# nihui/rife-ncnn-vulkan

Measured on AMD Instinct MI355X. Metric: interpolated frames/sec (rife-v4.6, 3840x2160), higher is better.
Workload: dtype f16x2-split MFMA + f32 accumulate (fp32-equivalent; activations stored f32 or as {hi, lo} f16 pairs); 1 GPU; rife-v4.6 3840x2160 frame pairs resident in HBM, timestep sweep [0.5, 0.125, 0.25, 0.7, 0.9], synthetic seeded weights; pairs_in_flight_per_gpu=4, cu_partition=every stream owns 1 / 2 of the compute units (rife_hip_stream_create), frames=F1: images/0.png, 1.png of the reference tiled 6 x 6, parallelism=frame pairs sharded over ranks, no data-path collective

## Files before the change

### rife-ncnn-vulkan_amd/csrc/conv_rs.h

```cpp
#pragma once
#include <type_traits>
#include "conv_t64.h"
#include "conv_row.h"

namespace rife {

constexpr int RS_NR = 12;
constexpr int RS_SEG = 34 * 32;
constexpr int RS_ROWB = 8 * RS_SEG;
constexpr int RS_STG_ROW = 8 * 1024;
constexpr int RS_LDS_RING = 0;
constexpr int RS_LDS_STG = RS_NR * RS_ROWB;
constexpr int RS_NSTG = 3;
constexpr int RS_LDS_BS = RS_LDS_STG + RS_NSTG * 2 * RS_STG_ROW;
constexpr int RS_LDS = RS_LDS_BS + 512;
constexpr int RS_AHEAD = 3;
constexpr int RS_MIN_PAIRS = 4;
constexpr int RS_NTHR = 512;

struct RsArgs {
    const unsigned char* in;
    unsigned char* out;
    const unsigned char* img;
    int H, W;
    int pitch;
    unsigned plane;
    int npairs;
    int nunits;
    int descend;
    long long* stamps = nullptr;
};
enum { RS_NOSTORE = 0x100, RS_NODMA = 0x200, RS_NOMATH = 0x400, RS_CLK = 0x40000, RS_PRIO = 0x2000, RS_NTLOAD = 0x4000, RS_NTSTORE = 0x8000 };

struct RsCursor {
    int strip, p;
    __device__ __forceinline__ void init(int u, int npairs) { strip = u / npairs; p = u - strip * npairs; }
    __device__ __forceinline__ bool advance(int npairs, int descend) {
        if (descend) { if (--p < 0) { p = npairs - 1; --strip; return true; } }
        else if (++p >= npairs) { p = 0; ++strip; return true; }
        return false;
    }
};

template <int TAG>
__device__ __forceinline__ void rs_dma16(const unsigned char* base, unsigned voff, unsigned dst) {
    unsigned keep;
    if RIFE_ABL(TAG & RS_NTLOAD)
        asm volatile("s_mov_b32 %0, m0\n\ts_mov_b32 m0, %2\n\ts_nop 0\n\tglobal_load_lds_dwordx4 %1, %3 nt\n\ts_mov_b32 m0, %0"
                     : "=&s"(keep) : "v"(voff), "s"(dst), "s"(base) : "memory");
    else
        asm volatile("s_mov_b32 %0, m0\n\ts_mov_b32 m0, %2\n\ts_nop 0\n\tglobal_load_lds_dwordx4 %1, %3\n\ts_mov_b32 m0, %0"
                     : "=&s"(keep) : "v"(voff), "s"(dst), "s"(base) : "memory");
}

#define RS_SYNC_LGKM() asm volatile("s_waitcnt lgkmcnt(0)\n\ts_barrier" ::: "memory")
#define RS_SYNC_VM(N) asm volatile("s_waitcnt vmcnt(" #N ")\n\ts_barrier" ::: "memory")
#define RS_SYNC_BARE() asm volatile("s_barrier" ::: "memory")

struct RsPairDesc { int c, t; bool idn; };
__host__ __device__ constexpr RsPairDesc rs_pair(int N, int m) {
    for (int c = 0; c < 4; c++) {
        const int cnt = 9 + ((c >> 1) == N ? 1 : 0);
        if (m < cnt) return m < 9 ? RsPairDesc{c, m, false} : RsPairDesc{c, 4, true};
        m -= cnt;
    }
    return RsPairDesc{0, 0, false};
}
constexpr int RS_NPAIR = 38, RS_PF = 3;

template <int N, int TAG>
__device__ __forceinline__ void rs_consumer(const RsArgs& a, unsigned char* const ldsb, const int ro, const int lane, const int S, const int ufirst) {
    const int h = lane >> 5, li = lane & 31;
    constexpr bool FAST = (TAG & S16_FAST) != 0;
    f16x8 W[4][9];
    {
        const unsigned char* wsrc = a.img + h * 1024 + (N * 32 + li) * 16;
#pragma unroll
        for (int c = 0; c < 4; c++)
#pragma unroll
            for (int t = 0; t < 9; t++) W[c][t] = *reinterpret_cast<const f16x8*>(wsrc + c * t64_wch(2) + t * 2048);
    }
    f16x8 idf[2];
    {
        const int ch = s16_row_channel(li);
#pragma unroll
        for (int hc = 0; hc < 2; hc++)
#pragma unroll
            for (int e = 0; e < 8; e++) idf[hc][e] = ch == 16 * hc + 8 * h + e ? (_Float16)1.f : (_Float16)0.f;
    }
    unsigned colo[3];
#pragma unroll
    for (int dx = 0; dx < 3; dx++) { const int px = li + dx; colo[dx] = (unsigned)(px * 32 + ((h ^ ((px >> 3) & 1)) << 4)); }
    unsigned char* const stg = ldsb + RS_LDS_STG + ro * RS_STG_ROW + ((2 * N + h) * 32 + li) * 64;
    const int qs = (li >> 1) & 3;

    RsCursor cur; cur.init(ufirst, a.npairs);
    int sq = 0;
    unsigned ad[9];
    auto step_addresses = [&](const bool fresh) {
        sq += fresh ? 4 : 2; if (sq >= RS_NR) sq -= RS_NR;
#pragma unroll
        for (int dy = 0; dy < 3; dy++) {
            const int j = ro + dy;
            int sl = a.descend ? sq + RS_NR - 1 - j : sq + RS_NR - 4 + j;
            if (sl >= RS_NR) sl -= RS_NR;
            const unsigned rb = (unsigned)(RS_LDS_RING + sl * RS_ROWB);
#pragma unroll
            for (int dx = 0; dx < 3; dx++) ad[dy * 3 + dx] = rb + colo[dx];
        }
    };
    constexpr int NF = RS_PF + 1;
    static_assert(NF == 4 && RS_NPAIR % NF == 2, "fragment set rotation across steps");
    f16x8 fh[NF], fl[NF];
    int it = 0;
    auto step = [&](auto par_c) {
        constexpr int PAR = decltype(par_c)::value;
        auto frag_read = [&](auto mc) {
            constexpr int m = decltype(mc)::value;
            constexpr RsPairDesc d = rs_pair(N, m % RS_NPAIR);
            constexpr int st = (m + 2 * PAR) % NF;
            fh[st] = *reinterpret_cast<const f16x8*>(ldsb + ad[d.t] + d.c * (2 * RS_SEG));
            if constexpr (!FAST || d.idn) fl[st] = *reinterpret_cast<const f16x8*>(ldsb + ad[d.t] + d.c * (2 * RS_SEG) + RS_SEG);
        };
        f32x16 accH, accL;
        if (!RIFE_ABL(TAG & RS_NOMATH)) {
            for_each_slot<0, RS_NPAIR>([&](auto mc) {
                constexpr int m = decltype(mc)::value;
                constexpr RsPairDesc d = rs_pair(N, m);
                constexpr int st = (m + 2 * PAR) % NF;
                if constexpr (m == RS_NPAIR - RS_PF) step_addresses(cur.advance(a.npairs, a.descend));
                frag_read(std::integral_constant<int, m + RS_PF>{});
                const f16x8 A = d.idn ? idf[d.c & 1] : W[d.c][d.t];
                if constexpr (FAST) {
                    if constexpr (m == 0) {
                        f32x16 z;
#pragma unroll
                        for (int q = 0; q < 16; q++) z[q] = 0.f;
                        accH = __builtin_amdgcn_mfma_f32_32x32x16_f16(A, fh[st], z, 0, 0, 0);
                    } else accH = __builtin_amdgcn_mfma_f32_32x32x16_f16(A, fh[st], accH, 0, 0, 0);
                    if constexpr (d.idn && (d.c & 1) == 0) {
                        f32x16 z;
#pragma unroll
                        for (int q = 0; q < 16; q++) z[q] = 0.f;
                        accL = __builtin_amdgcn_mfma_f32_32x32x16_f16(A, fl[st], z, 0, 0, 0);
                    } else if constexpr (d.idn) accL = __builtin_amdgcn_mfma_f32_32x32x16_f16(A, fl[st], accL, 0, 0, 0);
                } else
                if constexpr (m == 0) {
                    f32x16 z;
#pragma unroll
                    for (int q = 0; q < 16; q++) z[q] = 0.f;
                    accH = __builtin_amdgcn_mfma_f32_32x32x16_f16(A, fh[st], z, 0, 0, 0);
                    accL = __builtin_amdgcn_mfma_f32_32x32x16_f16(A, fl[st], z, 0, 0, 0);
                } else {
                    accH = __builtin_amdgcn_mfma_f32_32x32x16_f16(A, fh[st], accH, 0, 0, 0);
                    accL = __builtin_amdgcn_mfma_f32_32x32x16_f16(A, fl[st], accL, 0, 0, 0);
                }
                __builtin_amdgcn_sched_barrier(0);
            });
        } else {
#pragma unroll
            for (int q = 0; q < 16; q++) { accH[q] = (float)lane; accL[q] = 0.f; }
        }
        int sb = it % RS_NSTG;
        f32x4* const d4 = reinterpret_cast<f32x4*>(stg + sb * (2 * RS_STG_ROW));
#pragma unroll
        for (int q = 0; q < 4; q++) {
            f32x4 v;
#pragma unroll
            for (int k = 0; k < 4; k++) v[k] = accH[4 * q + k] + accL[4 * q + k];
            d4[q ^ qs] = v;
        }
        RS_SYNC_BARE();
        it++;
    };
    RS_SYNC_LGKM();
    step_addresses(true);
    if (!RIFE_ABL(TAG & RS_NOMATH)) for_each_slot<0, RS_PF>([&](auto mc) {
        constexpr int m = decltype(mc)::value;
        constexpr RsPairDesc d = rs_pair(N, m);
        fh[m % NF] = *reinterpret_cast<const f16x8*>(ldsb + ad[d.t] + d.c * (2 * RS_SEG));
        if constexpr (!FAST || d.idn) fl[m % NF] = *reinterpret_cast<const f16x8*>(ldsb + ad[d.t] + d.c * (2 * RS_SEG) + RS_SEG);
    });
    while (it + 1 < S) { step(std::integral_constant<int, 0>{}); step(std::integral_constant<int, 1>{}); }
    if (it < S) step(std::integral_constant<int, 0>{});
    RS_SYNC_LGKM();
}

template <int TAG, int SPLIT = 0>
__global__ __launch_bounds__(RS_NTHR) __attribute__((amdgpu_waves_per_eu(2, 2))) void conv_rs_kernel(RsArgs a) {
    extern __shared__ __attribute__((aligned(16))) unsigned char ldsb[];
    const int tid = threadIdx.x, lane = tid & 63;
    const int wv = __builtin_amdgcn_readfirstlane(tid >> 6);
    long long clk0 = 0, rt0 = 0;
    if RIFE_ABL(TAG & RS_CLK) { clk0 = (long long)__builtin_readcyclecounter(); rt0 = (long long)__builtin_amdgcn_s_memrealtime(); }

    const int nwg = gridDim.x, b = blockIdx.x;
    const int u0 = (int)((long long)a.nunits * b / nwg), u1 = (int)((long long)a.nunits * (b + 1) / nwg);
    const int S = u1 - u0;
    if (S <= 0) return;
    const int ufirst = a.descend ? u1 - 1 : u0;

    auto epilogue = [&](const int j, const int sb, const int cstrip, const int cp, const int cc0, const int cc1, const float slope) {
        const int px = lane >> 1, jh = lane & 1, qs = (px >> 1) & 3;
        const int y = 2 * cp + j, x0 = 32 * cstrip;
        if (!(y < a.H) || RIFE_ABL(TAG & RS_NOSTORE)) return;
        const unsigned okmask = x0 + px < a.W ? 0xffffffffu : 0u;
        const unsigned char* src = ldsb + RS_LDS_STG + sb * (2 * RS_STG_ROW) + j * RS_STG_ROW + px * 64;
        unsigned char* dst = a.out + ((unsigned)((y + 1) * a.pitch + x0 + 1) * 32u + (unsigned)(lane * 16));
        for (int cc = cc0; cc < cc1; cc++) {
            const f32x4 r0 = *reinterpret_cast<const f32x4*>(src + cc * 2048 + (((2 * jh) ^ qs) << 4));
            const f32x4 r1 = *reinterpret_cast<const f32x4*>(src + cc * 2048 + (((2 * jh + 1) ^ qs) << 4));
            const f32x4 b0 = *reinterpret_cast<const f32x4*>(ldsb + RS_LDS_BS + (16 * cc + 8 * jh) * 4);
            const f32x4 b1 = *reinterpret_cast<const f32x4*>(ldsb + RS_LDS_BS + (16 * cc + 8 * jh + 4) * 4);
            f16x8 hv, lv;
#pragma unroll
            for (int e = 0; e < 8; e++) {
                const float yv = (e < 4 ? r0[e & 3] : r1[e & 3]) + (e < 4 ? b0[e & 3] : b1[e & 3]);
                float v = yv < 0.f ? yv * slope : yv;
                v = __uint_as_float(__float_as_uint(v) & okmask);
                const _Float16 hh = (_Float16)v;
                hv[e] = hh;
                lv[e] = (_Float16)(v - (float)hh);
            }
            *reinterpret_cast<f16x8*>(dst + (size_t)(2 * cc) * a.plane) = hv;
            *reinterpret_cast<f16x8*>(dst + (size_t)(2 * cc + 1) * a.plane) = lv;
        }
    };
    if (wv < 4) {
        if RIFE_ABL(TAG & RS_PRIO) __builtin_amdgcn_s_setprio(2);
        if (wv == 0 && lane < 32) reinterpret_cast<f32x4*>(ldsb + RS_LDS_BS)[lane] = reinterpret_cast<const f32x4*>(a.img + 4 * t64_wch(2))[lane];
        if (wv & 1) rs_consumer<1, TAG>(a, ldsb, wv >> 1, lane, S, ufirst);
        else rs_consumer<0, TAG>(a, ldsb, wv >> 1, lane, S, ufirst);
    } else if (wv < 6) {
        const int j = wv - 4;
        unsigned soff[9];
#pragma unroll
        for (int i = 0; i < 9; i++) {
            const int u = min(i * 64 + lane, 543);
            const int seg = u / 68, within = u - seg * 68;
            const int px = within >> 1, pos = within & 1;
            const int kh = pos ^ ((px >> 3) & 1);
            soff[i] = (unsigned)seg * a.plane + (unsigned)(px * 32 + kh * 16);
        }
        RsCursor cur; cur.init(ufirst, a.npairs);
        int sq = 0;
        auto load_step = [&](bool fresh) -> int {
            const int nnew = fresh ? 4 : 2;
            const int y = 2 * cur.p, x0 = 32 * cur.strip;
            int mine = 0;
            for (int i = j; i < nnew; i += 2) {
                const int prow = a.descend ? y + nnew - 1 - i : y + 4 - nnew + i;
                int sl = sq + i; if (sl >= RS_NR) sl -= RS_NR;
                if (!RIFE_ABL(TAG & RS_NODMA)) {
                    const unsigned rowoff = (unsigned)(prow * a.pitch + x0) * 32u;
                    const unsigned dst = (unsigned)(RS_LDS_RING + sl * RS_ROWB);
#pragma unroll
                    for (int k = 0; k < 8; k++) rs_dma16<TAG>(a.in, rowoff + soff[k], dst + k * 1024);
                    if (lane < 32) rs_dma16<TAG>(a.in, rowoff + soff[8], dst + 8 * 1024);
                }
                mine += 9;
            }
            sq += nnew; if (sq >= RS_NR) sq -= RS_NR;
            return mine;
        };
        if RIFE_ABL(TAG & RS_NODMA) { for (int i = lane + 64 * j; i < RS_LDS_STG / 16; i += 128) reinterpret_cast<f32x4*>(ldsb)[i] = f32x4{0.f, 0.f, 0.f, 0.f}; }
        load_step(true);
        int ahead = 0;
        int loaded = 1;
        for (; loaded < RS_AHEAD && loaded < S; loaded++) { const bool f = cur.advance(a.npairs, a.descend); ahead = load_step(f); }
        if (loaded < RS_AHEAD) ahead = 0;
#define RS_WAIT_AHEAD()                                                                                      \
        if RIFE_ABL(TAG & RS_NODMA) RS_SYNC_LGKM();                                                                  \
        else if (ahead == 0) RS_SYNC_VM(0);                                                                  \
        else if (ahead == 9) RS_SYNC_VM(9);                                                                  \
        else RS_SYNC_VM(18);
        RS_WAIT_AHEAD()
        if (SPLIT) {
            const float slope = reinterpret_cast<const float*>(a.img + 4 * t64_wch(2))[64];
            RsCursor ecur; ecur.init(ufirst, a.npairs);
            for (int it = 0; it <= S + 1; it++) {
                if (it >= 2) { epilogue(j, (it - 2) % RS_NSTG, ecur.strip, ecur.p, 0, 2, slope); ecur.advance(a.npairs, a.descend); }
                if (it < S) {
                    if (it + RS_AHEAD < S) { const bool f = cur.advance(a.npairs, a.descend); ahead = load_step(f); }
                    else ahead = 0;
                    asm volatile("s_waitcnt lgkmcnt(0)" ::: "memory");
                    RS_WAIT_AHEAD()
                } else if (it == S) RS_SYNC_LGKM();
            }
        } else {
        for (int it = 0; it < S; it++) {
            if (it + RS_AHEAD < S) { const bool f = cur.advance(a.npairs, a.descend); ahead = load_step(f); }
            else ahead = 0;
            RS_WAIT_AHEAD()
        }
        RS_SYNC_BARE();
        }
#undef RS_WAIT_AHEAD
    } else {
        const int j = wv - 6;
        const int px = lane >> 1, jh = lane & 1, qs = (px >> 1) & 3;
        const float slope = reinterpret_cast<const float*>(a.img + 4 * t64_wch(2))[64];
        RsCursor cur; cur.init(ufirst, a.npairs);
        RS_SYNC_LGKM();
        for (int it = 0; it <= S + 1; it++) {
            if (it >= 2) {
                const int y = 2 * cur.p + j, x0 = 32 * cur.strip;
                if (SPLIT) epilogue(j, (it - 2) % RS_NSTG, cur.strip, cur.p, 2, 4, slope);
                else if (y < a.H && !RIFE_ABL(TAG & RS_NOSTORE)) {
                    const unsigned okmask = x0 + px < a.W ? 0xffffffffu : 0u;
                    const unsigned char* src = ldsb + RS_LDS_STG + ((it - 2) % RS_NSTG) * (2 * RS_STG_ROW) + j * RS_STG_ROW + px * 64;
                    unsigned char* dst = a.out + ((unsigned)((y + 1) * a.pitch + x0 + 1) * 32u + (unsigned)(lane * 16));
#pragma unroll
                    for (int cc = 0; cc < 4; cc++) {
                        const f32x4 r0 = *reinterpret_cast<const f32x4*>(src + cc * 2048 + (((2 * jh) ^ qs) << 4));
                        const f32x4 r1 = *reinterpret_cast<const f32x4*>(src + cc * 2048 + (((2 * jh + 1) ^ qs) << 4));
                        const f32x4 b0 = *reinterpret_cast<const f32x4*>(ldsb + RS_LDS_BS + (16 * cc + 8 * jh) * 4);
                        const f32x4 b1 = *reinterpret_cast<const f32x4*>(ldsb + RS_LDS_BS + (16 * cc + 8 * jh + 4) * 4);
                        f16x8 hv, lv;
#pragma unroll
                        for (int e = 0; e < 8; e++) {
                            const float yv = (e < 4 ? r0[e & 3] : r1[e & 3]) + (e < 4 ? b0[e & 3] : b1[e & 3]);
                            float v = yv < 0.f ? yv * slope : yv;
                            v = __uint_as_float(__float_as_uint(v) & okmask);
                            const _Float16 hh = (_Float16)v;
                            hv[e] = hh;
                            lv[e] = (_Float16)(v - (float)hh);
                        }
                        if RIFE_ABL(TAG & RS_NTSTORE) {
                            __builtin_nontemporal_store(hv, reinterpret_cast<f16x8*>(dst + (size_t)(2 * cc) * a.plane));
                            __builtin_nontemporal_store(lv, reinterpret_cast<f16x8*>(dst + (size_t)(2 * cc + 1) * a.plane));
                        } else {
                            *reinterpret_cast<f16x8*>(dst + (size_t)(2 * cc) * a.plane) = hv;
                            *reinterpret_cast<f16x8*>(dst + (size_t)(2 * cc + 1) * a.plane) = lv;
                        }
                    }
                }
                cur.advance(a.npairs, a.descend);
            }
            if (it < S) RS_SYNC_LGKM();
            else if (it == S) RS_SYNC_LGKM();
        }
    }
    if (RIFE_ABL(TAG & RS_CLK) && tid == 0) {
        a.stamps[4 * blockIdx.x] = (long long)__builtin_readcyclecounter() - clk0;
        a.stamps[4 * blockIdx.x + 1] = rt0;
        a.stamps[4 * blockIdx.x + 2] = (long long)__builtin_amdgcn_s_memrealtime();
    }
}

}
```

### rife-ncnn-vulkan_amd/csrc/conv_rs2.h

```cpp
#pragma once
#include "conv_rs.h"

namespace rife {

constexpr int RS2_SW = 30;
constexpr int RS2_NRA = 8;
constexpr int RS2_NRB = 5;
constexpr int RS2_AH = 3;
constexpr int RS2_NSTG = 3;
constexpr int RS2_LDS_RA = 0;
constexpr int RS2_LDS_RB = RS2_LDS_RA + RS2_NRA * RS_ROWB;
constexpr int RS2_LDS_SA = RS2_LDS_RB + RS2_NRB * RS_ROWB;
constexpr int RS2_LDS_SB = RS2_LDS_SA + RS2_NSTG * RS_STG_ROW;
constexpr int RS2_LDS_BS = RS2_LDS_SB + RS2_NSTG * RS_STG_ROW;
constexpr int RS2_LDS = RS2_LDS_BS + 1024;
static_assert(RS2_LDS <= 160 * 1024, "LDS budget of one CU");
static_assert(RS2_NRA == 4 + RS2_AH + 1, "the row issued in iteration it (sequence it + 4 + AH) takes the slot of row it - 1");
constexpr int RS2_NTHR = 512;
constexpr int RS2_MIN_ROWS = 8;

struct Rs2Args {
    const unsigned char* in;
    unsigned char* out;
    const unsigned char* imgA;
    const unsigned char* imgB;
    int H, W;
    int pitch;
    unsigned plane;
    int rowmax;
    int kparts;
    int nseg;
    int descend;
    int limit;
    long long* stamps = nullptr;
    int stamp_wg = 0;
};

struct Rs2Seg { int x0, ystart, dir, R; };
__device__ __forceinline__ Rs2Seg rs2_segment(const Rs2Args& a, const int seg) {
    const int strip = seg / a.kparts, part = seg - strip * a.kparts;
    const int r0 = (int)((long long)a.H * part / a.kparts), r1 = (int)((long long)a.H * (part + 1) / a.kparts);
    Rs2Seg s;
    s.x0 = RS2_SW * strip; s.R = r1 - r0; s.dir = a.descend ? -1 : 1; s.ystart = a.descend ? r1 - 1 : r0;
    return s;
}

#define RS2_NEXT(V, MOD) { V = V + 1 == (MOD) ? 0 : V + 1; }
enum { RS2_STAMPS = 0x1000, RS2_NOFRAG = 0x10, RS2_NOLO = 0x20 };
constexpr int RS2_NSTAMP = 128;
#define RS2_BAR(KIND)                                                                                                  \
    {                                                                                                                  \
        if (RIFE_ABL(TAG & RS2_STAMPS) && (int)blockIdx.x == a.stamp_wg && bar < RS2_NSTAMP && (threadIdx.x & 63) == 0)         \
            a.stamps[((threadIdx.x >> 6) * RS2_NSTAMP + bar) * 2] = (long long)__builtin_readcyclecounter();           \
        RS_SYNC_##KIND;                                                                                                \
        if (RIFE_ABL(TAG & RS2_STAMPS) && (int)blockIdx.x == a.stamp_wg && bar < RS2_NSTAMP && (threadIdx.x & 63) == 0)         \
            a.stamps[((threadIdx.x >> 6) * RS2_NSTAMP + bar) * 2 + 1] = (long long)__builtin_readcyclecounter();       \
        bar++;                                                                                                         \
    }

template <int N, int NR, int TAG>
__device__ __forceinline__ void rs2_consumer(const Rs2Args& a, const unsigned char* const img, unsigned char* const ldsb, const unsigned ring, const unsigned stgbase,
                                             const int lead, const int extra, const int lag, const int lane) {
    const int h = lane >> 5, li = lane & 31;
    constexpr bool FAST = (TAG & S16_FAST) != 0;
    f16x8 W[4][9];
    {
        const unsigned char* wsrc = img + h * 1024 + (N * 32 + li) * 16;
#pragma unroll
        for (int c = 0; c < 4; c++)
#pragma unroll
            for (int t = 0; t < 9; t++) W[c][t] = *reinterpret_cast<const f16x8*>(wsrc + c * t64_wch(2) + t * 2048);
    }
    f16x8 idf[2];
    {
        const int ch = s16_row_channel(li);
#pragma unroll
        for (int hc = 0; hc < 2; hc++)
#pragma unroll
            for (int e = 0; e < 8; e++) idf[hc][e] = ch == 16 * hc + 8 * h + e ? (_Float16)1.f : (_Float16)0.f;
    }
    unsigned colo[3];
#pragma unroll
    for (int dx = 0; dx < 3; dx++) { const int px = li + dx; colo[dx] = (unsigned)(px * 32 + ((h ^ ((px >> 3) & 1)) << 4)); }
    unsigned char* const stg = ldsb + stgbase + ((2 * N + h) * 32 + li) * 64;
    const int qs = (li >> 1) & 3;

    int bar = 0;
    int sq = 0;
    int sbuf = 0;
    unsigned ad[9];
    auto step_addresses = [&]() {
#pragma unroll
        for (int dy = 0; dy < 3; dy++) {
            int sl = sq + (a.descend ? 2 - dy : dy);
            if (sl >= NR) sl -= NR;
            const unsigned rb = ring + (unsigned)(sl * RS_ROWB);
#pragma unroll
            for (int dx = 0; dx < 3; dx++) ad[dy * 3 + dx] = rb + colo[dx];
        }
    };
    constexpr int NF = RS_PF + 1;
    static_assert(NF == 4 && RS_NPAIR % NF == 2, "fragment set rotation across steps");
    f16x8 fh[NF], fl[NF];
    auto step = [&](auto par_c) {
        constexpr int PAR = decltype(par_c)::value;
        auto frag_read = [&](auto mc) {
            constexpr int m = decltype(mc)::value;
            constexpr RsPairDesc d = rs_pair(N, m % RS_NPAIR);
            constexpr int st = (m + 2 * PAR) % NF;
            if RIFE_ABL(TAG & RS2_NOFRAG) { asm volatile("" : "+v"(fh[st]), "+v"(fl[st])); return; }
            fh[st] = *reinterpret_cast<const f16x8*>(ldsb + ad[d.t] + d.c * (2 * RS_SEG));
            if constexpr (FAST && !d.idn) return;
            if (!RIFE_ABL(TAG & RS2_NOLO)) fl[st] = *reinterpret_cast<const f16x8*>(ldsb + ad[d.t] + d.c * (2 * RS_SEG) + RS_SEG);
        };
        f32x16 accH, accL;
        if (!RIFE_ABL(TAG & RS_NOMATH)) {
            for_each_slot<0, RS_NPAIR>([&](auto mc) {
                constexpr int m = decltype(mc)::value;
                constexpr RsPairDesc d = rs_pair(N, m);
                constexpr int st = (m + 2 * PAR) % NF;
                if constexpr (m == RS_NPAIR - RS_PF) { RS2_NEXT(sq, NR) step_addresses(); }
                frag_read(std::integral_constant<int, m + RS_PF>{});
                const f16x8 A = d.idn ? idf[d.c & 1] : W[d.c][d.t];
                if constexpr (FAST) {
                    if constexpr (m == 0) {
                        f32x16 z;
#pragma unroll
                        for (int q = 0; q < 16; q++) z[q] = 0.f;
                        accH = __builtin_amdgcn_mfma_f32_32x32x16_f16(A, fh[st], z, 0, 0, 0);
                    } else accH = __builtin_amdgcn_mfma_f32_32x32x16_f16(A, fh[st], accH, 0, 0, 0);
                    if constexpr (d.idn && (d.c & 1) == 0) {
                        f32x16 z;
#pragma unroll
                        for (int q = 0; q < 16; q++) z[q] = 0.f;
                        accL = __builtin_amdgcn_mfma_f32_32x32x16_f16(A, fl[st], z, 0, 0, 0);
                    } else if constexpr (d.idn) accL = __builtin_amdgcn_mfma_f32_32x32x16_f16(A, fl[st], accL, 0, 0, 0);
                } else
                if constexpr (m == 0) {
                    f32x16 z;
#pragma unroll
                    for (int q = 0; q < 16; q++) z[q] = 0.f;
                    accH = __builtin_amdgcn_mfma_f32_32x32x16_f16(A, fh[st], z, 0, 0, 0);
                    if (!RIFE_ABL(TAG & RS2_NOLO)) accL = __builtin_amdgcn_mfma_f32_32x32x16_f16(A, fl[st], z, 0, 0, 0); else accL = z;
                } else {
                    accH = __builtin_amdgcn_mfma_f32_32x32x16_f16(A, fh[st], accH, 0, 0, 0);
                    if (!RIFE_ABL(TAG & RS2_NOLO)) accL = __builtin_amdgcn_mfma_f32_32x32x16_f16(A, fl[st], accL, 0, 0, 0);
                }
                __builtin_amdgcn_sched_barrier(0);
            });
        } else {
#pragma unroll
            for (int q = 0; q < 16; q++) { accH[q] = (float)lane; accL[q] = 0.f; }
        }
        f32x4* const d4 = reinterpret_cast<f32x4*>(stg + sbuf * RS_STG_ROW);
#pragma unroll
        for (int q = 0; q < 4; q++) {
            f32x4 v;
#pragma unroll
            for (int k = 0; k < 4; k++) v[k] = accH[4 * q + k] + accL[4 * q + k];
            d4[q ^ qs] = v;
        }
        RS2_NEXT(sbuf, RS2_NSTG)
        RS2_BAR(BARE())
    };
    for (int seg = blockIdx.x; seg < a.nseg; seg += gridDim.x) {
        const int R = rs2_segment(a, seg).R;
        const int S = R + extra, NIT = R + lag + 2;
        RS2_BAR(LGKM())
        for (int i = 0; i < lead; i++) RS2_BAR(BARE())
        sq = 0; sbuf = lead % RS2_NSTG;
        step_addresses();
        if (!RIFE_ABL(TAG & RS_NOMATH)) for_each_slot<0, RS_PF>([&](auto mc) {
            constexpr int m = decltype(mc)::value;
            constexpr RsPairDesc d = rs_pair(N, m);
            fh[m % NF] = *reinterpret_cast<const f16x8*>(ldsb + ad[d.t] + d.c * (2 * RS_SEG));
            if constexpr (!FAST || d.idn) fl[m % NF] = *reinterpret_cast<const f16x8*>(ldsb + ad[d.t] + d.c * (2 * RS_SEG) + RS_SEG);
        });
        int k = 0;
        for (; k + 1 < S; k += 2) { step(std::integral_constant<int, 0>{}); step(std::integral_constant<int, 1>{}); }
        if (k < S) step(std::integral_constant<int, 0>{});
        for (int i = lead + S; i < NIT; i++) RS2_BAR(BARE())
    }
}

__device__ __forceinline__ void rs2_finish(const unsigned char* const src, const unsigned char* const bs, const int cc, const int jh, const int qs, const float slope, const unsigned okmask,
                                           f16x8& hv, f16x8& lv) {
    const f32x4 r0 = *reinterpret_cast<const f32x4*>(src + cc * 2048 + (((2 * jh) ^ qs) << 4));
    const f32x4 r1 = *reinterpret_cast<const f32x4*>(src + cc * 2048 + (((2 * jh + 1) ^ qs) << 4));
    const f32x4 b0 = *reinterpret_cast<const f32x4*>(bs + (16 * cc + 8 * jh) * 4);
    const f32x4 b1 = *reinterpret_cast<const f32x4*>(bs + (16 * cc + 8 * jh + 4) * 4);
#pragma unroll
    for (int e = 0; e < 8; e++) {
        const float yv = (e < 4 ? r0[e & 3] : r1[e & 3]) + (e < 4 ? b0[e & 3] : b1[e & 3]);
        float v = yv < 0.f ? yv * slope : yv;
        v = __uint_as_float(__float_as_uint(v) & okmask);
        const _Float16 hh = (_Float16)v;
        hv[e] = hh;
        lv[e] = (_Float16)(v - (float)hh);
    }
}

template <int TAG>
__global__ __launch_bounds__(RS2_NTHR) __attribute__((amdgpu_waves_per_eu(2, 2))) void conv_rs2_kernel(Rs2Args a) {
    extern __shared__ __attribute__((aligned(16))) unsigned char ldsb[];
    const int tid = threadIdx.x, lane = tid & 63;
    const int wv = __builtin_amdgcn_readfirstlane(tid >> 6);
    long long clk0 = 0, rt0 = 0;
    if RIFE_ABL(TAG & RS_CLK) { clk0 = (long long)__builtin_readcyclecounter(); rt0 = (long long)__builtin_amdgcn_s_memrealtime(); }
    if ((int)blockIdx.x >= a.nseg) return;
    const int lag = a.descend ? 6 : 5;
    if (wv < 4) {
        if ((wv == 0 || wv == 2) && lane < 32)
            reinterpret_cast<f32x4*>(ldsb + RS2_LDS_BS + (wv >> 1) * 512)[lane] = reinterpret_cast<const f32x4*>((wv ? a.imgB : a.imgA) + 4 * t64_wch(2))[lane];
        if (wv == 0) rs2_consumer<0, RS2_NRA, TAG>(a, a.imgA, ldsb, RS2_LDS_RA, RS2_LDS_SA, 0, 2, lag, lane);
        else if (wv == 1) rs2_consumer<1, RS2_NRA, TAG>(a, a.imgA, ldsb, RS2_LDS_RA, RS2_LDS_SA, 0, 2, lag, lane);
        else if (wv == 2) rs2_consumer<0, RS2_NRB, TAG>(a, a.imgB, ldsb, RS2_LDS_RB, RS2_LDS_SB, lag, 0, lag, lane);
        else rs2_consumer<1, RS2_NRB, TAG>(a, a.imgB, ldsb, RS2_LDS_RB, RS2_LDS_SB, lag, 0, lag, lane);
    } else if (wv == 4) {
        int bar = 0;
        int soff[9];
#pragma unroll
        for (int i = 0; i < 9; i++) {
            const int u = min(i * 64 + lane, 543);
            const int sg = u / 68, within = u - sg * 68;
            const int px = within >> 1, pos = within & 1;
            const int kh = pos ^ ((px >> 3) & 1);
            soff[i] = (int)((unsigned)sg * a.plane) + px * 32 + kh * 16;
        }
        if RIFE_ABL(TAG & RS_NODMA) { for (int i = lane; i < RS2_LDS_SA / 16; i += 64) reinterpret_cast<f32x4*>(ldsb)[i] = f32x4{0.f, 0.f, 0.f, 0.f}; }
        for (int seg = blockIdx.x; seg < a.nseg; seg += gridDim.x) {
            const Rs2Seg s = rs2_segment(a, seg);
            const int needed = s.R + 4, NIT = s.R + lag + 2;
            int issued = 0;
            auto issue = [&]() {
                const int y = s.ystart + s.dir * (issued - 2);
                const int prow = min(max(y + 1, 0), a.H + 1);
                if (!RIFE_ABL(TAG & RS_NODMA)) {
                    const int rowoff = (prow * a.pitch + s.x0 - 1) * 32;
                    const unsigned dst = (unsigned)(RS2_LDS_RA + (issued & (RS2_NRA - 1)) * RS_ROWB);
#pragma unroll
                    for (int k = 0; k < 8; k++) rs_dma16<TAG>(a.in, (unsigned)min(max(rowoff + soff[k], 0), a.limit), dst + k * 1024);
                    if (lane < 32) rs_dma16<TAG>(a.in, (unsigned)min(max(rowoff + soff[8], 0), a.limit), dst + 8 * 1024);
                }
                issued++;
            };
            auto wait_barrier = [&](const int pending) {
                if RIFE_ABL(TAG & RS_NODMA) RS2_BAR(LGKM())
                else if (pending <= 0) RS2_BAR(VM(0))
                else if (pending == 1) RS2_BAR(VM(9))
                else if (pending == 2) RS2_BAR(VM(18))
                else RS2_BAR(VM(27))
            };
            static_assert(RS2_AH == 3, "counted waits above");
            while (issued < min(needed, 4 + RS2_AH)) issue();
            wait_barrier(issued - min(needed, 4));
            for (int it = 0; it < NIT; it++) {
                if (issued < needed) issue();
                wait_barrier(issued - min(needed, it + 5));
            }
        }
    } else if (wv < 7) {
        const int e = wv - 5;
        int bar = 0;
        const int px = lane >> 1, jh = lane & 1, qs = (px >> 1) & 3;
        const float slope = reinterpret_cast<const float*>(a.imgA + 4 * t64_wch(2))[64];
        const unsigned dcol = (unsigned)(px * 32 + ((jh ^ ((px >> 3) & 1)) << 4));
        for (int seg = blockIdx.x; seg < a.nseg; seg += gridDim.x) {
            const Rs2Seg s = rs2_segment(a, seg);
            const int NIT = s.R + lag + 2;
            RS2_BAR(LGKM())
            RS2_BAR(BARE()) RS2_BAR(BARE())
            int slot = 0, sb = 0;
            const int xA = s.x0 - 1 + px;
            const bool colok = xA >= 0 && xA < a.W;
            for (int j = 0; j < s.R + 2; j++) {
                const int yA = s.ystart + s.dir * (j - 1);
                const unsigned okmask = (colok && yA >= 0 && yA < a.H) ? 0xffffffffu : 0u;
                const unsigned char* src = ldsb + RS2_LDS_SA + sb * RS_STG_ROW + px * 64;
                unsigned char* dst = ldsb + RS2_LDS_RB + slot * RS_ROWB + dcol;
#pragma unroll
                for (int cc = 2 * e; cc < 2 * e + 2; cc++) {
                    f16x8 hv, lv;
                    rs2_finish(src, ldsb + RS2_LDS_BS, cc, jh, qs, slope, okmask, hv, lv);
                    *reinterpret_cast<f16x8*>(dst + (2 * cc) * RS_SEG) = hv;
                    *reinterpret_cast<f16x8*>(dst + (2 * cc + 1) * RS_SEG) = lv;
                }
                RS2_NEXT(slot, RS2_NRB) RS2_NEXT(sb, RS2_NSTG)
                RS2_BAR(LGKM())
            }
            for (int i = s.R + 4; i < NIT; i++) RS2_BAR(BARE())
        }
    } else {
        const int px = lane >> 1, jh = lane & 1, qs = (px >> 1) & 3;
        const float slope = reinterpret_cast<const float*>(a.imgB + 4 * t64_wch(2))[64];
        int bar = 0;
        for (int seg = blockIdx.x; seg < a.nseg; seg += gridDim.x) {
            const Rs2Seg s = rs2_segment(a, seg);
            RS2_BAR(LGKM())
            for (int i = 0; i < lag + 2; i++) RS2_BAR(BARE())
            int sb = lag % RS2_NSTG;
            const int x = s.x0 + px;
            const bool store = px < RS2_SW && x < a.rowmax && !RIFE_ABL(TAG & RS_NOSTORE);
            const unsigned okmask = x < a.W ? 0xffffffffu : 0u;
            for (int rho = 0; rho < s.R; rho++) {
                const int y = s.ystart + s.dir * rho;
                if (store) {
                    const unsigned char* src = ldsb + RS2_LDS_SB + sb * RS_STG_ROW + px * 64;
                    unsigned char* dst = a.out + ((unsigned)((y + 1) * a.pitch + s.x0 + 1) * 32u + (unsigned)(lane * 16));
#pragma unroll
                    for (int cc = 0; cc < 4; cc++) {
                        f16x8 hv, lv;
                        rs2_finish(src, ldsb + RS2_LDS_BS + 512, cc, jh, qs, slope, okmask, hv, lv);
                        *reinterpret_cast<f16x8*>(dst + (size_t)(2 * cc) * a.plane) = hv;
                        *reinterpret_cast<f16x8*>(dst + (size_t)(2 * cc + 1) * a.plane) = lv;
                    }
                }
                RS2_NEXT(sb, RS2_NSTG)
                RS2_BAR(LGKM())
            }
        }
    }
    if (RIFE_ABL(TAG & RS_CLK) && tid == 0) {
        a.stamps[4 * blockIdx.x] = (long long)__builtin_readcyclecounter() - clk0;
        a.stamps[4 * blockIdx.x + 1] = rt0;
        a.stamps[4 * blockIdx.x + 2] = (long long)__builtin_amdgcn_s_memrealtime();
    }
}

}
```

Baseline: 520.2 frames/s.

## Switch row-stream conv consumer from 32x32x16 to 16x16x32 MFMA with new fragment layout

```diff
diff --git a/rife-ncnn-vulkan_amd/csrc/conv_rs.h b/rife-ncnn-vulkan_amd/csrc/conv_rs.h
--- a/rife-ncnn-vulkan_amd/csrc/conv_rs.h
+++ b/rife-ncnn-vulkan_amd/csrc/conv_rs.h
@@ -2,6 +2,7 @@
 #include <type_traits>
 #include "conv_t64.h"
 #include "conv_row.h"
+#include "rs_frag_geom.h"
 
 namespace rife {
 
@@ -17,6 +18,8 @@
 constexpr int RS_AHEAD = 3;
 constexpr int RS_MIN_PAIRS = 4;
 constexpr int RS_NTHR = 512;
+static_assert(RS_SEG == rsg::SEG && RS_ROWB == rsg::ROWB && RS_STG_ROW == rsg::STG_ROW && t64_wch(2) == rsg::WCH && rsg::IMG_W < T64_IMG, "rs_frag_geom.h restates these");
+static_assert(s16_row_channel(5) == rsg::row_channel(5) && s16_row_channel(26) == rsg::row_channel(26), "rs_frag_geom.h restates s16_row_channel");
 
 struct RsArgs {
     const unsigned char* in;
@@ -57,46 +60,94 @@
 #define RS_SYNC_VM(N) asm volatile("s_waitcnt vmcnt(" #N ")\n\ts_barrier" ::: "memory")
 #define RS_SYNC_BARE() asm volatile("s_barrier" ::: "memory")
 
-struct RsPairDesc { int c, t; bool idn; };
-__host__ __device__ constexpr RsPairDesc rs_pair(int N, int m) {
-    for (int c = 0; c < 4; c++) {
-        const int cnt = 9 + ((c >> 1) == N ? 1 : 0);
-        if (m < cnt) return m < 9 ? RsPairDesc{c, m, false} : RsPairDesc{c, 4, true};
-        m -= cnt;
-    }
-    return RsPairDesc{0, 0, false};
-}
-constexpr int RS_NPAIR = 38, RS_PF = 3;
+constexpr int RS_NPAIR = rsg::NUNIT, RS_PF = 3;
+enum { RS2_NOFRAG = 0x10, RS2_NOLO = 0x20 };
+
+template <int N, int TAG>
+struct RsRow {
+    static constexpr bool FAST = (TAG & S16_FAST) != 0;
+    static constexpr int NF = RS_PF + 1;
+    static_assert(NF == 4 && RS_NPAIR % NF == 2, "fragment set rotation across steps");
+    f16x8 W[2][9][2], idf[2];
+    f16x8 fh[NF], fl[NF];
+    f32x4 acc[2][2][2];
+    unsigned colo[3];
+    unsigned ad[9];
+    unsigned stgo;
+
+    __device__ __forceinline__ void init(const unsigned char* const img, const int lane) {
+#pragma unroll
+        for (int half = 0; half < 2; half++) {
+            const unsigned char* const wsrc = img + rsg::w_lane(lane, N, half);
+#pragma unroll
+            for (int cp = 0; cp < 2; cp++)
+#pragma unroll
+                for (int t = 0; t < 9; t++) W[cp][t][half] = *reinterpret_cast<const f16x8*>(wsrc + rsg::w_frag(cp, t));
+#pragma unroll
+            for (int j = 0; j < 8; j++) idf[half][j] = rsg::id_one(lane, half, j) ? (_Float16)1.f : (_Float16)0.f;
+        }
+#pragma unroll
+        for (int dx = 0; dx < 3; dx++) colo[dx] = (unsigned)rsg::pix_lane(lane, dx);
+        stgo = (unsigned)rsg::stg_lane(lane, N);
+    }
+    __device__ __forceinline__ void set_row(const int dy, const unsigned rb) {
+#pragma unroll
+        for (int dx = 0; dx < 3; dx++) ad[dy * 3 + dx] = rb + colo[dx];
+    }
+    template <int M, int PAR>
+    __device__ __forceinline__ void read(const unsigned char* const ldsb) {
+        constexpr rsg::Unit u = rsg::unit(N, M % RS_NPAIR);
+        constexpr int st = (M + 2 * PAR) % NF;
+        if RIFE_ABL(TAG & RS2_NOFRAG) { asm volatile("" : "+v"(fh[st]), "+v"(fl[st])); return; }
+        fh[st] = *reinterpret_cast<const f16x8*>(ldsb + ad[u.t] + rsg::pix_frag(u.cp, 0, u.ph));
+        if constexpr (FAST && !u.idn) return;
+        if (!RIFE_ABL(TAG & RS2_NOLO)) fl[st] = *reinterpret_cast<const f16x8*>(ldsb + ad[u.t] + rsg::pix_frag(u.cp, 1, u.ph));
+    }
+    __device__ __forceinline__ void read_first(const unsigned char* const ldsb) {
+        for_each_slot<0, RS_PF>([&](auto mc) { read<decltype(mc)::value, 0>(ldsb); });
+    }
+    template <int PAR, class NEXT>
+    __device__ __forceinline__ void products(const unsigned char* const ldsb, NEXT&& next) {
+        for_each_slot<0, RS_NPAIR>([&](auto mc) {
+            constexpr int m = decltype(mc)::value;
+            constexpr rsg::Unit u = rsg::unit(N, m);
+            constexpr int st = (m + 2 * PAR) % NF;
+            constexpr bool open = !u.idn && u.cp == 0 && u.t == 0;
+            if constexpr (m == RS_NPAIR - RS_PF) next();
+            read<m + RS_PF, PAR>(ldsb);
+            const f32x4 z = {0.f, 0.f, 0.f, 0.f};
+#pragma unroll
+            for (int half = 0; half < 2; half++) {
+                const f16x8 A = u.idn ? idf[half] : W[u.cp][u.t][half];
+                acc[0][half][u.ph] = __builtin_amdgcn_mfma_f32_16x16x32_f16(A, fh[st], open ? z : acc[0][half][u.ph], 0, 0, 0);
+                if constexpr (FAST) {
+                    if constexpr (u.idn) acc[1][half][u.ph] = __builtin_amdgcn_mfma_f32_16x16x32_f16(A, fl[st], z, 0, 0, 0);
+                } else if (!RIFE_ABL(TAG & RS2_NOLO)) acc[1][half][u.ph] = __builtin_amdgcn_mfma_f32_16x16x32_f16(A, fl[st], open ? z : acc[1][half][u.ph], 0, 0, 0);
+                else if constexpr (open) acc[1][half][u.ph] = z;
+            }
+            __builtin_amdgcn_sched_barrier(0);
+        });
+    }
+    __device__ __forceinline__ void fill(const float v) {
+#pragma unroll
+        for (int i = 0; i < 4; i++) { acc[0][i >> 1][i & 1] = f32x4{v, v, v, v}; acc[1][i >> 1][i & 1] = f32x4{0.f, 0.f, 0.f, 0.f}; }
+    }
+    __device__ __forceinline__ void stage(unsigned char* const row) {
+#pragma unroll
+        for (int half = 0; half < 2; half++)
+#pragma unroll
+            for (int ph = 0; ph < 2; ph++) *reinterpret_cast<f32x4*>(row + stgo + rsg::stg_tile(half, ph)) = acc[0][half][ph] + acc[1][half][ph];
+    }
+};
 
 template <int N, int TAG>
 __device__ __forceinline__ void rs_consumer(const RsArgs& a, unsigned char* const ldsb, const int ro, const int lane, const int S, const int ufirst) {
-    const int h = lane >> 5, li = lane & 31;
-    constexpr bool FAST = (TAG & S16_FAST) != 0;
-    f16x8 W[4][9];
-    {
-        const unsigned char* wsrc = a.img + h * 1024 + (N * 32 + li) * 16;
-#pragma unroll
-        for (int c = 0; c < 4; c++)
-#pragma unroll
-            for (int t = 0; t < 9; t++) W[c][t] = *reinterpret_cast<const f16x8*>(wsrc + c * t64_wch(2) + t * 2048);
-    }
-    f16x8 idf[2];
-    {
-        const int ch = s16_row_channel(li);
-#pragma unroll
-        for (int hc = 0; hc < 2; hc++)
-#pragma unroll
-            for (int e = 0; e < 8; e++) idf[hc][e] = ch == 16 * hc + 8 * h + e ? (_Float16)1.f : (_Float16)0.f;
-    }
-    unsigned colo[3];
-#pragma unroll
-    for (int dx = 0; dx < 3; dx++) { const int px = li + dx; colo[dx] = (unsigned)(px * 32 + ((h ^ ((px >> 3) & 1)) << 4)); }
-    unsigned char* const stg = ldsb + RS_LDS_STG + ro * RS_STG_ROW + ((2 * N + h) * 32 + li) * 64;
-    const int qs = (li >> 1) & 3;
+    RsRow<N, TAG> row;
+    row.init(a.img, lane);
+    unsigned char* const stg = ldsb + RS_LDS_STG + ro * RS_STG_ROW;
 
     RsCursor cur; cur.init(ufirst, a.npairs);
     int sq = 0;
-    unsigned ad[9];
     auto step_addresses = [&](const bool fresh) {
         sq += fresh ? 4 : 2; if (sq >= RS_NR) sq -= RS_NR;
 #pragma unroll
@@ -104,83 +155,21 @@
             const int j = ro + dy;
             int sl = a.descend ? sq + RS_NR - 1 - j : sq + RS_NR - 4 + j;
             if (sl >= RS_NR) sl -= RS_NR;
-            const unsigned rb = (unsigned)(RS_LDS_RING + sl * RS_ROWB);
-#pragma unroll
-            for (int dx = 0; dx < 3; dx++) ad[dy * 3 + dx] = rb + colo[dx];
+            row.set_row(dy, (unsigned)(RS_LDS_RING + sl * RS_ROWB));
         }
     };
-    constexpr int NF = RS_PF + 1;
-    static_assert(NF == 4 && RS_NPAIR % NF == 2, "fragment set rotation across steps");
-    f16x8 fh[NF], fl[NF];
     int it = 0;
     auto step = [&](auto par_c) {
         constexpr int PAR = decltype(par_c)::value;
-        auto frag_read = [&](auto mc) {
-            constexpr int m = decltype(mc)::value;
-            constexpr RsPairDesc d = rs_pair(N, m % RS_NPAIR);
-            constexpr int st = (m + 2 * PAR) % NF;
-            fh[st] = *reinterpret_cast<const f16x8*>(ldsb + ad[d.t] + d.c * (2 * RS_SEG));
-            if constexpr (!FAST || d.idn) fl[st] = *reinterpret_cast<const f16x8*>(ldsb + ad[d.t] + d.c * (2 * RS_SEG) + RS_SEG);
-        };
-        f32x16 accH, accL;
-        if (!RIFE_ABL(TAG & RS_NOMATH)) {
-            for_each_slot<0, RS_NPAIR>([&](auto mc) {
-                constexpr int m = decltype(mc)::value;
-                constexpr RsPairDesc d = rs_pair(N, m);
-                constexpr int st = (m + 2 * PAR) % NF;
-                if constexpr (m == RS_NPAIR - RS_PF) step_addresses(cur.advance(a.npairs, a.descend));
-                frag_read(std::integral_constant<int, m + RS_PF>{});
-                const f16x8 A = d.idn ? idf[d.c & 1] : W[d.c][d.t];
-                if constexpr (FAST) {
-                    if constexpr (m == 0) {
-                        f32x16 z;
-#pragma unroll
-                        for (int q = 0; q < 16; q++) z[q] = 0.f;
-                        accH = __builtin_amdgcn_mfma_f32_32x32x16_f16(A, fh[st], z, 0, 0, 0);
-                    } else accH = __builtin_amdgcn_mfma_f32_32x32x16_f16(A, fh[st], accH, 0, 0, 0);
-                    if constexpr (d.idn && (d.c & 1) == 0) {
-                        f32x16 z;
-#pragma unroll
-                        for (int q = 0; q < 16; q++) z[q] = 0.f;
-                        accL = __builtin_amdgcn_mfma_f32_32x32x16_f16(A, fl[st], z, 0, 0, 0);
-                    } else if constexpr (d.idn) accL = __builtin_amdgcn_mfma_f32_32x32x16_f16(A, fl[st], accL, 0, 0, 0);
-                } else
-                if constexpr (m == 0) {
-                    f32x16 z;
-#pragma unroll
-                    for (int q = 0; q < 16; q++) z[q] = 0.f;
-                    accH = __builtin_amdgcn_mfma_f32_32x32x16_f16(A, fh[st], z, 0, 0, 0);
-                    accL = __builtin_amdgcn_mfma_f32_32x32x16_f16(A, fl[st], z, 0, 0, 0);
-                } else {
-                    accH = __builtin_amdgcn_mfma_f32_32x32x16_f16(A, fh[st], accH, 0, 0, 0);
-                    accL = __builtin_amdgcn_mfma_f32_32x32x16_f16(A, fl[st], accL, 0, 0, 0);
-                }
-                __builtin_amdgcn_sched_barrier(0);
-            });
-        } else {
-#pragma unroll
-            for (int q = 0; q < 16; q++) { accH[q] = (float)lane; accL[q] = 0.f; }
-        }
-        int sb = it % RS_NSTG;
-        f32x4* const d4 = reinterpret_cast<f32x4*>(stg + sb * (2 * RS_STG_ROW));
-#pragma unroll
-        for (int q = 0; q < 4; q++) {
-            f32x4 v;
-#pragma unroll
-            for (int k = 0; k < 4; k++) v[k] = accH[4 * q + k] + accL[4 * q + k];
-            d4[q ^ qs] = v;
-        }
+        if (!RIFE_ABL(TAG & RS_NOMATH)) row.template products<PAR>(ldsb, [&]() { step_addresses(cur.advance(a.npairs, a.descend)); });
+        else row.fill((float)lane);
+        row.stage(stg + (it % RS_NSTG) * (2 * RS_STG_ROW));
         RS_SYNC_BARE();
         it++;
     };
     RS_SYNC_LGKM();
     step_addresses(true);
-    if (!RIFE_ABL(TAG & RS_NOMATH)) for_each_slot<0, RS_PF>([&](auto mc) {
-        constexpr int m = decltype(mc)::value;
-        constexpr RsPairDesc d = rs_pair(N, m);
-        fh[m % NF] = *reinterpret_cast<const f16x8*>(ldsb + ad[d.t] + d.c * (2 * RS_SEG));
-        if constexpr (!FAST || d.idn) fl[m % NF] = *reinterpret_cast<const f16x8*>(ldsb + ad[d.t] + d.c * (2 * RS_SEG) + RS_SEG);
-    });
+    if (!RIFE_ABL(TAG & RS_NOMATH)) row.read_first(ldsb);
     while (it + 1 < S) { step(std::integral_constant<int, 0>{}); step(std::integral_constant<int, 1>{}); }
     if (it < S) step(std::integral_constant<int, 0>{});
     RS_SYNC_LGKM();
@@ -239,8 +228,7 @@
             const int u = min(i * 64 + lane, 543);
             const int seg = u / 68, within = u - seg * 68;
             const int px = within >> 1, pos = within & 1;
-            const int kh = pos ^ ((px >> 3) & 1);
-            soff[i] = (unsigned)seg * a.plane + (unsigned)(px * 32 + kh * 16);
+            soff[i] = (unsigned)seg * a.plane + (unsigned)(px * 32 + pos * 16);
         }
         RsCursor cur; cur.init(ufirst, a.npairs);
         int sq = 0;
diff --git a/rife-ncnn-vulkan_amd/csrc/conv_rs2.h b/rife-ncnn-vulkan_amd/csrc/conv_rs2.h
--- a/rife-ncnn-vulkan_amd/csrc/conv_rs2.h
+++ b/rife-ncnn-vulkan_amd/csrc/conv_rs2.h
@@ -46,7 +46,7 @@
 }
 
 #define RS2_NEXT(V, MOD) { V = V + 1 == (MOD) ? 0 : V + 1; }
-enum { RS2_STAMPS = 0x1000, RS2_NOFRAG = 0x10, RS2_NOLO = 0x20 };
+enum { RS2_STAMPS = 0x1000 };
 constexpr int RS2_NSTAMP = 128;
 #define RS2_BAR(KIND)                                                                                                  \
     {                                                                                                                  \
@@ -61,105 +61,26 @@
 template <int N, int NR, int TAG>
 __device__ __forceinline__ void rs2_consumer(const Rs2Args& a, const unsigned char* const img, unsigned char* const ldsb, const unsigned ring, const unsigned stgbase,
                                              const int lead, const int extra, const int lag, const int lane) {
-    const int h = lane >> 5, li = lane & 31;
-    constexpr bool FAST = (TAG & S16_FAST) != 0;
-    f16x8 W[4][9];
-    {
-        const unsigned char* wsrc = img + h * 1024 + (N * 32 + li) * 16;
-#pragma unroll
-        for (int c = 0; c < 4; c++)
-#pragma unroll
-            for (int t = 0; t < 9; t++) W[c][t] = *reinterpret_cast<const f16x8*>(wsrc + c * t64_wch(2) + t * 2048);
-    }
-    f16x8 idf[2];
-    {
-        const int ch = s16_row_channel(li);
-#pragma unroll
-        for (int hc = 0; hc < 2; hc++)
-#pragma unroll
-            for (int e = 0; e < 8; e++) idf[hc][e] = ch == 16 * hc + 8 * h + e ? (_Float16)1.f : (_Float16)0.f;
-    }
-    unsigned colo[3];
-#pragma unroll
-    for (int dx = 0; dx < 3; dx++) { const int px = li + dx; colo[dx] = (unsigned)(px * 32 + ((h ^ ((px >> 3) & 1)) << 4)); }
-    unsigned char* const stg = ldsb + stgbase + ((2 * N + h) * 32 + li) * 64;
-    const int qs = (li >> 1) & 3;
+    RsRow<N, TAG> row;
+    row.init(img, lane);
+    unsigned char* const stg = ldsb + stgbase;
 
     int bar = 0;
     int sq = 0;
     int sbuf = 0;
-    unsigned ad[9];
     auto step_addresses = [&]() {
 #pragma unroll
         for (int dy = 0; dy < 3; dy++) {
             int sl = sq + (a.descend ? 2 - dy : dy);
             if (sl >= NR) sl -= NR;
-            const unsigned rb = ring + (unsigned)(sl * RS_ROWB);
-#pragma unroll
-            for (int dx = 0; dx < 3; dx++) ad[dy * 3 + dx] = rb + colo[dx];
+            row.set_row(dy, ring + (unsigned)(sl * RS_ROWB));
         }
     };
-    constexpr int NF = RS_PF + 1;
-    static_assert(NF == 4 && RS_NPAIR % NF == 2, "fragment set rotation across steps");
-    f16x8 fh[NF], fl[NF];
     auto step = [&](auto par_c) {
         constexpr int PAR = decltype(par_c)::value;
-        auto frag_read = [&](auto mc) {
-            constexpr int m = decltype(mc)::value;
-            constexpr RsPairDesc d = rs_pair(N, m % RS_NPAIR);
-            constexpr int st = (m + 2 * PAR) % NF;
-            if RIFE_ABL(TAG & RS2_NOFRAG) { asm volatile("" : "+v"(fh[st]), "+v"(fl[st])); return; }
-            fh[st] = *reinterpret_cast<const f16x8*>(ldsb + ad[d.t] + d.c * (2 * RS_SEG));
-            if constexpr (FAST && !d.idn) return;
-            if (!RIFE_ABL(TAG & RS2_NOLO)) fl[st] = *reinterpret_cast<const f16x8*>(ldsb + ad[d.t] + d.c * (2 * RS_SEG) + RS_SEG);
-        };
-        f32x16 accH, accL;
-        if (!RIFE_ABL(TAG & RS_NOMATH)) {
-            for_each_slot<0, RS_NPAIR>([&](auto mc) {
-                constexpr int m = decltype(mc)::value;
-                constexpr RsPairDesc d = rs_pair(N, m);
-                constexpr int st = (m + 2 * PAR) % NF;
-                if constexpr (m == RS_NPAIR - RS_PF) { RS2_NEXT(sq, NR) step_addresses(); }
-                frag_read(std::integral_constant<int, m + RS_PF>{});
-                const f16x8 A = d.idn ? idf[d.c & 1] : W[d.c][d.t];
-                if constexpr (FAST) {
-                    if constexpr (m == 0) {
-                        f32x16 z;
-#pragma unroll
-                        for (int q = 0; q < 16; q++) z[q] = 0.f;
-                        accH = __builtin_amdgcn_mfma_f32_32x32x16_f16(A, fh[st], z, 0, 0, 0);
-                    } else accH = __builtin_amdgcn_mfma_f32_32x32x16_f16(A, fh[st], accH, 0, 0, 0);
-                    if constexpr (d.idn && (d.c & 1) == 0) {
-                        f32x16 z;
-#pragma unroll
-                        for (int q = 0; q < 16; q++) z[q] = 0.f;
-                        accL = __builtin_amdgcn_mfma_f32_32x32x16_f16(A, fl[st], z, 0, 0, 0);
-                    } else if constexpr (d.idn) accL = __builtin_amdgcn_mfma_f32_32x32x16_f16(A, fl[st], accL, 0, 0, 0);
-                } else
-                if constexpr (m == 0) {
-                    f32x16 z;
-#pragma unroll
-                    for (int q = 0; q < 16; q++) z[q] = 0.f;
-                    accH = __builtin_amdgcn_mfma_f32_32x32x16_f16(A, fh[st], z, 0, 0, 0);
-                    if (!RIFE_ABL(TAG & RS2_NOLO)) accL = __builtin_amdgcn_mfma_f32_32x32x16_f16(A, fl[st], z, 0, 0, 0); else accL = z;
-                } else {
-                    accH = __builtin_amdgcn_mfma_f32_32x32x16_f16(A, fh[st], accH, 0, 0, 0);
-                    if (!RIFE_ABL(TAG & RS2_NOLO)) accL = __builtin_amdgcn_mfma_f32_32x32x16_f16(A, fl[st], accL, 0, 0, 0);
-                }
-                __builtin_amdgcn_sched_barrier(0);
-            });
-        } else {
-#pragma unroll
-            for (int q = 0; q < 16; q++) { accH[q] = (float)lane; accL[q] = 0.f; }
-        }
-        f32x4* const d4 = reinterpret_cast<f32x4*>(stg + sbuf * RS_STG_ROW);
-#pragma unroll
-        for (int q = 0; q < 4; q++) {
-            f32x4 v;
-#pragma unroll
-            for (int k = 0; k < 4; k++) v[k] = accH[4 * q + k] + accL[4 * q + k];
-            d4[q ^ qs] = v;
-        }
+        if (!RIFE_ABL(TAG & RS_NOMATH)) row.template products<PAR>(ldsb, [&]() { RS2_NEXT(sq, NR) step_addresses(); });
+        else row.fill((float)lane);
+        row.stage(stg + sbuf * RS_STG_ROW);
         RS2_NEXT(sbuf, RS2_NSTG)
         RS2_BAR(BARE())
     };
@@ -170,12 +91,7 @@
         for (int i = 0; i < lead; i++) RS2_BAR(BARE())
         sq = 0; sbuf = lead % RS2_NSTG;
         step_addresses();
-        if (!RIFE_ABL(TAG & RS_NOMATH)) for_each_slot<0, RS_PF>([&](auto mc) {
-            constexpr int m = decltype(mc)::value;
-            constexpr RsPairDesc d = rs_pair(N, m);
-            fh[m % NF] = *reinterpret_cast<const f16x8*>(ldsb + ad[d.t] + d.c * (2 * RS_SEG));
-            if constexpr (!FAST || d.idn) fl[m % NF] = *reinterpret_cast<const f16x8*>(ldsb + ad[d.t] + d.c * (2 * RS_SEG) + RS_SEG);
-        });
+        if (!RIFE_ABL(TAG & RS_NOMATH)) row.read_first(ldsb);
         int k = 0;
         for (; k + 1 < S; k += 2) { step(std::integral_constant<int, 0>{}); step(std::integral_constant<int, 1>{}); }
         if (k < S) step(std::integral_constant<int, 0>{});
@@ -224,8 +140,7 @@
             const int u = min(i * 64 + lane, 543);
             const int sg = u / 68, within = u - sg * 68;
             const int px = within >> 1, pos = within & 1;
-            const int kh = pos ^ ((px >> 3) & 1);
-            soff[i] = (int)((unsigned)sg * a.plane) + px * 32 + kh * 16;
+            soff[i] = (int)((unsigned)sg * a.plane) + px * 32 + pos * 16;
         }
         if RIFE_ABL(TAG & RS_NODMA) { for (int i = lane; i < RS2_LDS_SA / 16; i += 64) reinterpret_cast<f32x4*>(ldsb)[i] = f32x4{0.f, 0.f, 0.f, 0.f}; }
         for (int seg = blockIdx.x; seg < a.nseg; seg += gridDim.x) {
@@ -264,7 +179,7 @@
         int bar = 0;
         const int px = lane >> 1, jh = lane & 1, qs = (px >> 1) & 3;
         const float slope = reinterpret_cast<const float*>(a.imgA + 4 * t64_wch(2))[64];
-        const unsigned dcol = (unsigned)(px * 32 + ((jh ^ ((px >> 3) & 1)) << 4));
+        const unsigned dcol = (unsigned)(px * 32 + jh * 16);
         for (int seg = blockIdx.x; seg < a.nseg; seg += gridDim.x) {
             const Rs2Seg s = rs2_segment(a, seg);
             const int NIT = s.R + lag + 2;
diff --git a/rife-ncnn-vulkan_amd/csrc/rs_frag_geom.h b/rife-ncnn-vulkan_amd/csrc/rs_frag_geom.h
--- /dev/null
+++ b/rife-ncnn-vulkan_amd/csrc/rs_frag_geom.h
@@ -0,0 +1,56 @@
+#pragma once
+
+#if defined(__HIPCC__)
+#define RSG_HD __host__ __device__
+#else
+#define RSG_HD
+#endif
+
+namespace rsg {
+
+constexpr int SEG = 34 * 32;
+constexpr int ROWB = 8 * SEG;
+constexpr int WCH = 9 * 2 * 64 * 16;
+constexpr int IMG_W = 4 * WCH;
+constexpr int STG_ROW = 8 * 1024;
+constexpr int NUNIT = 38;
+
+RSG_HD constexpr int row_channel(int i) { return 16 * ((i >> 2) & 1) + 4 * (i >> 3) + (i & 3); }
+RSG_HD constexpr int channel_row(int ch) { return 8 * ((ch >> 2) & 3) + 4 * (ch >> 4) + (ch & 3); }
+
+RSG_HD constexpr int lane_col(int l) { return l & 15; }
+RSG_HD constexpr int lane_kg(int l) { return l >> 4; }
+RSG_HD constexpr int kg_chunk(int kg) { return kg >> 1; }
+RSG_HD constexpr int kg_half(int kg) { return kg & 1; }
+
+struct Unit { int cp, t, ph; bool idn; };
+RSG_HD constexpr Unit unit(int N, int m) {
+    for (int cp = 0; cp < 2; cp++) {
+        const int cnt = 18 + (cp == N ? 2 : 0);
+        if (m < cnt) return m < 18 ? Unit{cp, m >> 1, m & 1, false} : Unit{cp, 4, m & 1, true};
+        m -= cnt;
+    }
+    return Unit{0, 0, 0, false};
+}
+
+RSG_HD constexpr int pix_lane(int l, int dx) { return (lane_col(l) + dx) * 32 + kg_chunk(lane_kg(l)) * (2 * SEG) + kg_half(lane_kg(l)) * 16; }
+RSG_HD constexpr int pix_frag(int cp, int plane, int ph) { return cp * (4 * SEG) + plane * SEG + ph * 512; }
+RSG_HD constexpr int pix_offset(int l, int dx, int cp, int plane, int ph) { return pix_lane(l, dx) + pix_frag(cp, plane, ph); }
+
+RSG_HD constexpr int w_lane(int l, int N, int half) {
+    return kg_chunk(lane_kg(l)) * WCH + kg_half(lane_kg(l)) * 1024 + (32 * N + channel_row(16 * half + lane_col(l))) * 16;
+}
+RSG_HD constexpr int w_frag(int cp, int t) { return 2 * cp * WCH + t * 2048; }
+RSG_HD constexpr int w_offset(int l, int N, int cp, int t, int half) { return w_lane(l, N, half) + w_frag(cp, t); }
+
+RSG_HD constexpr bool id_one(int l, int half, int j) { return 8 * lane_kg(l) + j == 16 * half + lane_col(l); }
+
+RSG_HD constexpr int stg_lane(int l, int N) { return (2 * N * 32 + lane_col(l)) * 64 + ((lane_kg(l) ^ ((lane_col(l) >> 1) & 3)) << 4); }
+RSG_HD constexpr int stg_tile(int half, int ph) { return half * 2048 + ph * 1024; }
+RSG_HD constexpr int stg_offset(int l, int N, int half, int ph) { return stg_lane(l, N) + stg_tile(half, ph); }
+
+static_assert((2 * SEG) % 256 == 128, "the second chunk of a pair sits in the other half of the LDS banks");
+static_assert(unit(0, 18).idn && unit(0, 19).ph == 1 && unit(0, 20).cp == 1 && !unit(0, 37).idn && unit(1, 36).idn && unit(1, 37).idn, "unit order");
+static_assert(channel_row(row_channel(13)) == 13 && row_channel(channel_row(29)) == 29, "inverse");
+
+}
```

After: 527.4 frames/s (median of 6 runs). 1.4% higher.
